# MohammadJohari/myslam

Hardware: AMD Instinct MI355X
Metric: ray.samples/s (render+bwd) (higher is better)
Workload: dtype f32; 1 GPU; BASELINE configs[1]: Replica room0 (synthetic), 4096 rays x 64 samples (56+8); mapping iteration: sample + render fwd + loss + bwd (planes+decoders), no optimiser; rays_of_the_job=4096, rays_this_rank=4096, samples_per_ray=64, plane_bytes=27147008, planes_layout=channels_last, parallelism=single GPU, launch=hipGraph replay of the captured iteration

## Files before the change

### include/eslam_hip.h

```cpp
#ifndef ESLAM_HIP_H
#define ESLAM_HIP_H

#include <stdint.h>

#ifdef __cplusplus
extern "C" {
#endif

#define ESLAM_ABI_VERSION 5
#define ESLAM_C_DIM 32
#define ESLAM_HIDDEN 16
#define ESLAM_FEAT (2 * ESLAM_C_DIM)
#define ESLAM_N_PLANES 12
#define ESLAM_MAX_SAMPLES 256
#define ESLAM_RAY_ORDERS 3
#define ESLAM_RAY_ORDER_WORDS(R) (ESLAM_RAY_ORDERS * (int64_t)(R) + 4)
#define ESLAM_N_DEC_PARAMS (2 * (16 * 64 + 16 + 16 * 16 + 16) + (1 * 16 + 1) + (3 * 16 + 3))

typedef void* eslam_stream_t;

typedef struct {
    const float* data;
    float* grad;
    int32_t h, w;
// ... 48 lines not shown
                           const uint32_t* rng_state, int64_t ray_offset, float* z_vals, eslam_stream_t stream);

int eslam_render_fwd(const eslam_plane_t* planes, const eslam_decoders_t* dec, const float* bound6_host,
                     const float* rays_o, const float* rays_d, const float* z_vals, int R, int S, float* depth,
                     float* rgb, float* sdf, float* raw_rgb, float* feat, const int32_t* ray_order,
                     uint32_t* rng_bump, eslam_stream_t stream);

int eslam_render_fwd_loss(const eslam_plane_t* planes, const eslam_decoders_t* dec, const float* bound6_host,
                          const float* rays_o, const float* rays_d, const float* z_vals, int R, int S, float* depth,
                          float* rgb, float* sdf, float* raw_rgb, float* feat, const int32_t* ray_order,
                          const float* gt_depth, const float* gt_color, double truncation, const float* weights5_host,
                          const uint8_t* ray_mask, float* scratch, float* acc, float* loss, uint32_t* rng_bump,
                          eslam_stream_t stream);

int eslam_planes_to_half(const eslam_plane_t* planes, eslam_stream_t stream);

int eslam_planes_relayout(const eslam_plane_t* src, const eslam_plane_t* dst, int field, eslam_stream_t stream);

int eslam_render_fwd_lowp(const eslam_plane_t* planes_f16, const eslam_decoders_t* dec, const float* bound6_host,
                          const float* rays_o, const float* rays_d, const float* z_vals, int R, int S, float* depth,
                          float* rgb, float* sdf, eslam_stream_t stream);

int eslam_ray_order(const float* rays_o, const float* rays_d, int R, int32_t* perm, eslam_stream_t stream);

int64_t eslam_bwd_workspace_bytes(int64_t n_points);

int eslam_render_bwd(const eslam_plane_t* planes, const eslam_decoders_t* dec, const float* bound6_host,
                     const float* rays_o, const float* rays_d, const float* z_vals, int R, int S,
                     const float* sdf, const float* raw_rgb, const float* feat, const float* g_depth,
                     const float* g_rgb, const float* g_sdf, float* g_dec, float* g_beta, float* g_rays_o,
                     float* g_rays_d, const int32_t* ray_order, void* workspace, eslam_stream_t stream);

int eslam_render_bwd_loss(const eslam_plane_t* planes, const eslam_decoders_t* dec, const float* bound6_host,
                          const float* rays_o, const float* rays_d, const float* z_vals, int R, int S,
                          const float* sdf, const float* raw_rgb, const float* feat, const float* depth,
                          const float* rgb, const float* gt_depth, const float* gt_color, double truncation,
                          const float* weights5_host, const uint8_t* ray_mask, const float* acc,
                          const float* upstream, float* loss_out, const float* g_depth, const float* g_rgb,
                          const float* g_sdf, float* g_dec, float* g_beta, float* g_rays_o, float* g_rays_d,
                          const int32_t* ray_order, void* workspace, eslam_stream_t stream);

int64_t eslam_saved_hidden_floats(int64_t R, int S);
int eslam_render_fwd_h(const eslam_plane_t* planes, const eslam_decoders_t* dec, const float* bound6_host,
                       const float* rays_o, const float* rays_d, const float* z_vals, int R, int S, float* depth,
                       float* rgb, float* sdf, float* raw_rgb, float* feat, const int32_t* ray_order,
                       uint32_t* rng_bump, float* hidden, eslam_stream_t stream);
// ... 224 lines not shown
```

### myslam_amd/_hip.py

```python
import ctypes
import os
import threading

import torch

_HERE = os.path.dirname(os.path.abspath(__file__))
LIB_PATH = os.environ.get("ESLAM_HIP_LIB") or os.path.join(_HERE, "lib", "libeslam_hip.so")

ABI_VERSION = 5
RAY_ORDERS = 3


def ray_order_words(R):
    return RAY_ORDERS * int(R) + 4
N_DEC_PARAMS = 2692
N_PLANES = 12


class PlaneDesc(ctypes.Structure):
    _fields_ = [("data", ctypes.c_void_p), ("grad", ctypes.c_void_p), ("h", ctypes.c_int32), ("w", ctypes.c_int32),
                ("stride_c", ctypes.c_int64), ("stride_y", ctypes.c_int64), ("stride_x", ctypes.c_int64),
                ("data_f16", ctypes.c_void_p)]


# ... 38 lines not shown
    "eslam_aabb_exit": (_i, [_vp, _vp, _i, _BP, _vp, _vp]),
    "eslam_sample_z": (_i, [_vp, _i, _i, _i, _d, _vp, _vp, _vp, _vp, _vp]),
    "eslam_importance_z": (_i, [_PP, _DP, _BP, _vp, _vp, _vp, _i, _i, _i, _vp, _vp, _vp, _vp, _vp]),
    "eslam_sample_z_all": (_i, [_PP, _DP, _BP, _vp, _vp, _vp, _i, _i, _i, _d, _vp, _vp, _vp, _vp, _vp, _vp, _vp]),
    "eslam_sample_z_all_rng": (_i, [_PP, _DP, _BP, _vp, _vp, _vp, _i, _i, _i, _d, _vp, _vp, _i, ctypes.c_uint64, _vp, _i64, _vp, _vp]),
    "eslam_loss_set_sizes": (_i, [_vp, _vp, _i, _i, _i, _d, _vp, _vp, _vp, _i, ctypes.c_uint64, _vp, _vp, _vp, _vp]),
    "eslam_mark_rays": (_i, [_PP, _BP, _vp, _vp, _vp, _i, _d, _vp, _i64, _vp, _vp]),
    "eslam_blocks_compact_scratch_words": (_i64, [_i64]),
    "eslam_blocks_compact": (_i, [_vp, _i64, _vp, _vp, _vp, _vp, _i, _vp]),
    "eslam_host_meta_alloc": (_i, [ctypes.POINTER(ctypes.c_void_p), ctypes.POINTER(ctypes.c_void_p)]),
    "eslam_host_meta_free": (_i, [_vp]),
    "eslam_shard_prologue": (_i, [_vp, _vp, _vp, _i64, _vp, _i64, _vp, _vp, _vp, _vp, _i, _i, _i, _d, _vp, _vp, _i, ctypes.c_uint64,
                                  _vp, _vp, _vp, _PP, _BP, _vp, _i64, _vp, _vp]),
    "eslam_blocks_pack_dev": (_i, [_vp, _vp, _vp, _i64, _vp, _i64, _i64, _vp, _vp, _vp]),
    "eslam_blocks_unpack_dev": (_i, [_vp, _vp, _vp, _i64, _vp, _i64, _i64, _vp, _vp]),
    "eslam_blocks_zero_dev": (_i, [_vp, _vp, _vp, _i64, _vp, _i64, _vp]),
    "eslam_render_fwd": (_i, [_PP, _DP, _BP, _vp, _vp, _vp, _i, _i, _vp, _vp, _vp, _vp, _vp, _vp, _vp, _vp]),
    "eslam_render_fwd_loss": (_i, [_PP, _DP, _BP, _vp, _vp, _vp, _i, _i, _vp, _vp, _vp, _vp, _vp, _vp, _vp, _vp, _d, _BP, _vp,
                                   _vp, _vp, _vp, _vp, _vp]),
    "eslam_planes_to_half": (_i, [_PP, _vp]),
    "eslam_planes_relayout": (_i, [_PP, _PP, _i, _vp]),
    "eslam_render_fwd_lowp": (_i, [_PP, _DP, _BP, _vp, _vp, _vp, _i, _i, _vp, _vp, _vp, _vp]),
    "eslam_ray_order": (_i, [_vp, _vp, _i, _vp, _vp]),
    "eslam_stream_wait": (_i, [_vp, _vp]),
    "eslam_zero_async": (_i, [_vp, _i64, _vp]),
    "eslam_bwd_workspace_bytes": (_i64, [_i64]),
    "eslam_render_bwd": (_i, [_PP, _DP, _BP, _vp, _vp, _vp, _i, _i, _vp, _vp, _vp, _vp, _vp, _vp, _vp, _vp, _vp, _vp,
                              _vp, _vp, _vp]),
    "eslam_render_bwd_loss": (_i, [_PP, _DP, _BP, _vp, _vp, _vp, _i, _i, _vp, _vp, _vp, _vp, _vp, _vp, _vp, _d, _BP, _vp, _vp,
                                   _vp, _vp, _vp, _vp, _vp, _vp, _vp, _vp, _vp, _vp, _vp, _vp]),
    "eslam_saved_hidden_floats": (_i64, [_i64, _i]),
    "eslam_render_fwd_h": (_i, [_PP, _DP, _BP, _vp, _vp, _vp, _i, _i, _vp, _vp, _vp, _vp, _vp, _vp, _vp, _vp, _vp]),
    "eslam_render_fwd_loss_h": (_i, [_PP, _DP, _BP, _vp, _vp, _vp, _i, _i, _vp, _vp, _vp, _vp, _vp, _vp, _vp, _vp, _d, _BP, _vp,
                                     _vp, _vp, _vp, _vp, _vp, _vp]),
    "eslam_render_bwd_h": (_i, [_PP, _DP, _BP, _vp, _vp, _vp, _i, _i, _vp, _vp, _vp, _vp, _vp, _vp, _vp, _vp, _vp, _vp,
                                _vp, _vp, _vp, _vp]),
    "eslam_render_bwd_loss_h": (_i, [_PP, _DP, _BP, _vp, _vp, _vp, _i, _i, _vp, _vp, _vp, _vp, _vp, _vp, _vp, _d, _BP, _vp, _vp,
                                     _vp, _vp, _vp, _vp, _vp, _vp, _vp, _vp, _vp, _vp, _vp, _vp, _vp]),
    "eslam_decode_fwd": (_i, [_PP, _DP, _BP, _vp, _i64, _i, _vp, _vp, _vp]),
    "eslam_sdf_grid": (_i, [_PP, _DP, _BP, _vp, _vp, _vp, _i64, _i64, _i64, _vp, _i, _i, _vp, _vp]),
    "eslam_mc_workspace_bytes": (_i64, [_i64, _i64, _i64]),
    "eslam_mc_count": (_i, [_vp, _i64, _i64, _i64, _f, _vp, _vp, _vp]),
    "eslam_mc_emit": (_i, [_vp, _i64, _i64, _i64, _f, ctypes.POINTER(_d), ctypes.POINTER(_d), _vp, _i64, _i64, _vp, _vp, _vp]),
    "eslam_mc_count_masked": (_i, [_vp, _vp, _i64, _i64, _i64, _f, _vp, _vp, _vp]),
    "eslam_tsdf_integrate": (_i, [_vp, _vp, _vp, _i64, _i64, _i64, ctypes.POINTER(_f), _f, _f, _vp, _vp, _vp, _vp, _i, _i, _i,
                                  _f, _f, _f, _f, _vp]),
# ... 254 lines not shown
```

### myslam_amd/csrc/eslam_sample.hip

```cpp
#include "eslam_decode_tile.h"

#pragma clang fp contract(off)

__device__ __forceinline__ void pixel_dir(float u, float v, float fx, float fy, float cx, float cy, float d[3]) {
    d[0] = __fdiv_rn(__fsub_rn(u, cx), fx);
    d[1] = -__fdiv_rn(__fsub_rn(v, cy), fy);
    d[2] = -1.0f;
}

__device__ __forceinline__ void rotate_dir(const float* __restrict__ c2w, const float d[3], float out[3]) {
#pragma unroll
    for (int j = 0; j < 3; ++j)
        out[j] = __fadd_rn(__fadd_rn(__fmul_rn(d[0], c2w[4 * j + 0]), __fmul_rn(d[1], c2w[4 * j + 1])),
                           __fmul_rn(d[2], c2w[4 * j + 2]));
}

__global__ void sample_rays_kernel(const int64_t* __restrict__ indices, int b, int n, int H0, int H1, int W0, int W1,
                                   int H, int W, float fx, float fy, float cx, float cy,
                                   const float* __restrict__ c2ws, const float* __restrict__ depths,
                                   const float* __restrict__ colors, float* __restrict__ rays_o,
                                   float* __restrict__ rays_d, float* __restrict__ depth, float* __restrict__ color) {
    const int i = blockIdx.x * blockDim.x + threadIdx.x;
    if (i >= b * n) return;
    const int img = i / n;
// ... 202 lines not shown
        zs[pos] = val;
    }
    WAVE_SYNC();
    for (int i = lane; i < S; i += WAVE)
        out[i] = t_rand ? jitter_one(zs, i, S, t_rand[(int64_t)ray * S + i])
                        : (rng.on && rng.perturb) ? jitter_one(zs, i, S, rng_uniform(rng, 0u, (rng.ray_offset + (uint32_t)ray) * (uint32_t)S + (uint32_t)i)) : zs[i];
}

__global__ __launch_bounds__(256) void sample_z_kernel(const float* __restrict__ gt_depth, int R, int n_strat,
                                                       int n_imp, float c15, float c3,
                                                       const float* __restrict__ t_free,
                                                       const float* __restrict__ t_surf,
                                                       const float* __restrict__ t_rand, float* __restrict__ z_vals) {
    __shared__ float zs_all[4][ESLAM_MAX_SAMPLES];
    const int lane = threadIdx.x & 63, wave = threadIdx.x >> 6;
    const int ray = blockIdx.x * 4 + wave;
    if (ray >= R) return;
    const float d = gt_depth[ray];
    if (!(d > 0.0f)) return;
    depth_guided_row(d, ray, n_strat, n_imp, c15, c3, t_free, t_surf, t_rand, z_vals + (int64_t)ray * (n_strat + n_imp), zs_all[wave], lane,
                     Rng{0u, 0u, false, false, 0u});
}

template <bool CL, bool WITH_DEPTH>
__global__ __launch_bounds__(256, 2) void importance_z_kernel(const PlaneSet planes, const eslam_decoders_t dec,
                                                           const Bound bnd, const float* __restrict__ rays_o,
                                                           const float* __restrict__ rays_d,
                                                           const float* __restrict__ gt_depth, int R, int n_strat,
                                                           int n_imp, const float* __restrict__ t_free,
                                                           const float* __restrict__ t_rand_uni,
                                                           const float* __restrict__ u_rand,
                                                           float* __restrict__ z_vals, float c15, float c3,
                                                           const float* __restrict__ t_surf,
                                                           const float* __restrict__ t_rand, const RngArg rng_arg) {
    const Rng rng = make_rng(rng_arg);
    __shared__ __attribute__((aligned(16))) float wlds[DEC_LDS];
    __shared__ float zu[ESLAM_MAX_SAMPLES];
    __shared__ float wt[ESLAM_MAX_SAMPLES];
    __shared__ float zn[ESLAM_MAX_SAMPLES];
    __shared__ float al[ESLAM_MAX_SAMPLES];
    const int lane = threadIdx.x & 63, wave = threadIdx.x >> 6;
    const int ray = blockIdx.x;
    const float d0 = gt_depth[ray];
    if (d0 > 0.0f) {
        if (WITH_DEPTH && wave == 0)
            depth_guided_row(d0, ray, n_strat, n_imp, c15, c3, t_free, t_surf, t_rand, z_vals + (int64_t)ray * (n_strat + n_imp), zu, lane, rng);
        return;
    }
    stage_decoder_weights_one(wlds, dec, 0, threadIdx.x, blockDim.x);
    const int r = lane & 15, q = lane >> 4;
    const int gp = gather_point<CL>(lane), gq = gather_piece<CL>(lane);
    const float beta = dec.beta[0];
    const int S = n_strat + n_imp;
    const float o[3] = {rays_o[3 * ray], rays_o[3 * ray + 1], rays_o[3 * ray + 2]};
    const float d[3] = {rays_d[3 * ray], rays_d[3 * ray + 1], rays_d[3 * ray + 2]};
    const float far = __fadd_rn(aabb_exit_dev(o, d, bnd), 0.01f);

    for (int i = threadIdx.x; i < n_strat; i += 256) {
        const float t = t_free[i];
        wt[i] = __fadd_rn(__fmul_rn(0.0f, __fsub_rn(1.0f, t)), __fmul_rn(far, t));
    }
    __syncthreads();
    for (int i = threadIdx.x; i < n_strat; i += 256)
        zu[i] = t_rand_uni ? jitter_one(wt, i, n_strat, t_rand_uni[(int64_t)ray * n_strat + i])
                           : (rng.on && rng.perturb) ? jitter_one(wt, i, n_strat, rng_uniform(rng, 1u, (rng.ray_offset + (uint32_t)ray) * (uint32_t)n_strat + (uint32_t)i)) : wt[i];
    __syncthreads();

    const int nblk = (n_strat + 15) >> 4;
#pragma unroll 1
    for (int b = wave; b < nblk; b += 4) {
        const int oz0 = opaque_zero(b);
        const float z = zu[min(16 * b + gp, n_strat - 1)];
// ... 60 lines not shown
    float* out_row = z_vals + (int64_t)ray * S;
    bool inversion = false;
    for (int i = lane; i + 1 < n_strat; i += WAVE) inversion |= !(zu[i] <= zu[i + 1]);
    const bool zu_sorted = __ballot(inversion) == 0ull;
    for (int i = lane; i < S; i += WAVE) {
        const float v = (i < n_strat) ? zu[i] : zn[i - n_strat];
        int pos = 0;
        if (zu_sorted) {
            if (i < n_strat) {
                pos = i;
                for (int j = 0; j < n_imp; ++j) pos += (zn[j] < v) ? 1 : 0;
            } else {
                const int j0 = i - n_strat;
                pos = count_le_sorted(zu, n_strat, v);
                for (int j = 0; j < n_imp; ++j) pos += (zn[j] < v || (zn[j] == v && j < j0)) ? 1 : 0;
            }
        } else {
            for (int k = 0; k < S; ++k) {
                const float o2 = (k < n_strat) ? zu[k] : zn[k - n_strat];
                pos += (o2 < v || (!(v < o2) && k < i)) ? 1 : 0;
            }
        }
        out_row[pos] = v;
    }
}


#include "eslam_loss_final.h"
#include "eslam_shard_dev.h"
struct SetSizesArgs {
    const float* gt_depth;
    const uint8_t* ray_mask;
    int R, n_strat, n_imp;
    float c15, c3;
    const float* t_free;
    const float* t_surf;
    const float* t_rand;
    RngArg rng;
    Trunc tr;
    unsigned* scratch;
    float* acc_out;
};
__device__ __forceinline__ void set_sizes_block(const SetSizesArgs& a, const int bid, const int nblocks) {
    const Rng rng = make_rng(a.rng);
    __shared__ float zs_all[4][ESLAM_MAX_SAMPLES];
    __shared__ float zo_all[4][ESLAM_MAX_SAMPLES];
// ... 163 lines not shown

extern "C" int eslam_importance_z(const eslam_plane_t* planes, const eslam_decoders_t* dec, const float* bound6_host,
                                  const float* rays_o, const float* rays_d, const float* gt_depth, int R, int n_strat,
                                  int n_imp, const float* t_free, const float* t_rand_uni, const float* u,
                                  float* z_vals, eslam_stream_t stream) {
    if (R <= 0) return 0;
    if (n_strat < 3 || n_imp < 0 || n_strat + n_imp > ESLAM_MAX_SAMPLES) {
        eslam_set_error("eslam_importance_z: n_strat=%d n_imp=%d unsupported", n_strat, n_imp);
        return 1;
    }
    if (!planes || !dec || !bound6_host || !rays_o || !rays_d || !gt_depth || !t_free || (n_imp > 0 && !u) || !z_vals) {
        eslam_set_error("eslam_importance_z: null argument");
        return 1;
    }
    if (eslam_validate_planes(planes, 0, 6)) return 1;
    PlaneSet ps;
    for (int i = 0; i < NPL; ++i) ps.p[i] = planes[i < 6 ? i : i - 6];
    const Bound bnd = make_bound(bound6_host);
    dim3 grid(R), block(256);
    eslam_prof_begin(PROF_IMPORTANCE_Z, (hipStream_t)stream);
    if (eslam_planes_channels_last(planes, 0, 6))
        hipLaunchKernelGGL((importance_z_kernel<true, false>), grid, block, 0, (hipStream_t)stream, ps, *dec, bnd, rays_o,
                           rays_d, gt_depth, R, n_strat, n_imp, t_free, t_rand_uni, u, z_vals, 0.0f, 0.0f,
                           (const float*)nullptr, (const float*)nullptr, RngArg{});
    else
        hipLaunchKernelGGL((importance_z_kernel<false, false>), grid, block, 0, (hipStream_t)stream, ps, *dec, bnd, rays_o,
                           rays_d, gt_depth, R, n_strat, n_imp, t_free, t_rand_uni, u, z_vals, 0.0f, 0.0f,
                           (const float*)nullptr, (const float*)nullptr, RngArg{});
    eslam_prof_end(PROF_IMPORTANCE_Z, (hipStream_t)stream);
    return eslam_check_launch("importance_z_kernel");
}

static int sample_z_all_impl(const char* who, const eslam_plane_t* planes, const eslam_decoders_t* dec,
                             const float* bound6_host, const float* rays_o, const float* rays_d, const float* gt_depth,
                             int R, int n_strat, int n_imp, double truncation, const float* t_free, const float* t_surf,
                             const float* t_rand, const float* t_rand_uni, const float* u, const RngArg rng,
                             float* z_vals, eslam_stream_t stream) {
    if (R <= 0) return 0;
    if (n_strat < 3 || n_imp < 0 || n_strat + n_imp > ESLAM_MAX_SAMPLES) {
        eslam_set_error("%s: n_strat=%d n_imp=%d unsupported", who, n_strat, n_imp);
        return 1;
    }
    if (!planes || !dec || !bound6_host || !rays_o || !rays_d || !gt_depth || !t_free ||
        (n_imp > 0 && ((!u && !rng.on) || !t_surf)) || !z_vals) {
        eslam_set_error("%s: null argument", who);
        return 1;
    }
    if ((int64_t)R * (n_strat + n_imp) >= ((int64_t)1 << 32)) {
        eslam_set_error("%s: batch too large", who);
        return 1;
    }
    if (eslam_validate_planes(planes, 0, 6)) return 1;
    PlaneSet ps;
    for (int i = 0; i < NPL; ++i) ps.p[i] = planes[i < 6 ? i : i - 6];
    const Bound bnd = make_bound(bound6_host);
    const float c15 = (float)(1.5 * truncation);
    const float c3 = (float)(3.0 * truncation);
    dim3 grid(R), block(256);
    eslam_prof_begin(PROF_SAMPLE_Z, (hipStream_t)stream);
    if (eslam_planes_channels_last(planes, 0, 6))
        hipLaunchKernelGGL((importance_z_kernel<true, true>), grid, block, 0, (hipStream_t)stream, ps, *dec, bnd, rays_o,
                           rays_d, gt_depth, R, n_strat, n_imp, t_free, t_rand_uni, u, z_vals, c15, c3, t_surf, t_rand, rng);
    else
        hipLaunchKernelGGL((importance_z_kernel<false, true>), grid, block, 0, (hipStream_t)stream, ps, *dec, bnd, rays_o,
                           rays_d, gt_depth, R, n_strat, n_imp, t_free, t_rand_uni, u, z_vals, c15, c3, t_surf, t_rand, rng);
    eslam_prof_end(PROF_SAMPLE_Z, (hipStream_t)stream);
    return eslam_check_launch("importance_z_kernel<with depth>");
}

extern "C" int eslam_sample_z_all(const eslam_plane_t* planes, const eslam_decoders_t* dec, const float* bound6_host,
                                  const float* rays_o, const float* rays_d, const float* gt_depth, int R, int n_strat,
                                  int n_imp, double truncation, const float* t_free, const float* t_surf,
                                  const float* t_rand, const float* t_rand_uni, const float* u, float* z_vals,
                                  eslam_stream_t stream) {
    return sample_z_all_impl("eslam_sample_z_all", planes, dec, bound6_host, rays_o, rays_d, gt_depth, R, n_strat, n_imp,
                             truncation, t_free, t_surf, t_rand, t_rand_uni, u, RngArg{}, z_vals, stream);
}

extern "C" int eslam_sample_z_all_rng(const eslam_plane_t* planes, const eslam_decoders_t* dec, const float* bound6_host,
                                      const float* rays_o, const float* rays_d, const float* gt_depth, int R, int n_strat,
                                      int n_imp, double truncation, const float* t_free, const float* t_surf, int perturb,
                                      uint64_t seed, const uint32_t* rng_state, int64_t ray_offset, float* z_vals,
                                      eslam_stream_t stream) {
    if (ray_offset < 0 || (ray_offset + (int64_t)(R > 0 ? R : 0)) * (n_strat + n_imp) >= ((int64_t)1 << 32)) {
        eslam_set_error("eslam_sample_z_all_rng: ray_offset %lld out of range", (long long)ray_offset);
        return 1;
    }
    RngArg rng;
// ... 88 lines not shown
```

### myslam_amd/csrc/eslam_scatter.hip

```cpp
#include <mutex>
#include <type_traits>
#include "eslam_decode_tile.h"
#include "eslam_dec_reduce.h"

#define SORT_MAX 8192
typedef float float2_t __attribute__((ext_vector_type(2)));

__device__ __forceinline__ unsigned spread3(unsigned v) {
    v &= 0x3FFu;
    v = (v | (v << 16)) & 0x030000FFu;
    v = (v | (v << 8)) & 0x0300F00Fu;
    v = (v | (v << 4)) & 0x030C30C3u;
    v = (v | (v << 2)) & 0x09249249u;
    return v;
}

#define ORD_BITS 5
#define ORD_CELLS (1 << (3 * ORD_BITS))
#define ORD_PER_THREAD (SORT_MAX / 1024)
__global__ __launch_bounds__(1024) void ray_order_kernel(const float* __restrict__ rays_o,
                                                         const float* __restrict__ rays_d, int R,
                                                         int* __restrict__ perm, int key_bits) {
    extern __shared__ __attribute__((aligned(16))) unsigned hist[];
    const int nwords = (1 << key_bits) >> 1;
    const int mbits = key_bits / 3;
    __shared__ float red[16][6];
    __shared__ float red2[16][11];
    __shared__ unsigned wsum[16];
    constexpr int NCAM_MAX = 32;
    __shared__ unsigned long long cam_bits[SORT_MAX / 64];
    __shared__ unsigned cam_before[SORT_MAX / 64 + 1];
    __shared__ float cam_dir[NCAM_MAX][3];
    __shared__ unsigned cam_ext[NCAM_MAX][2];
    const int tid = threadIdx.x, lane = tid & 63, wave = tid >> 6;
    if (tid < SORT_MAX / 64) cam_bits[tid] = 0ull;
    if (tid < NCAM_MAX) { cam_dir[tid][0] = cam_dir[tid][1] = cam_dir[tid][2] = 0.f; cam_ext[tid][0] = 0xFFFFFFFFu; cam_ext[tid][1] = 0u; }
    __syncthreads();
    const int base = blockIdx.x * SORT_MAX;
    const int n = min(SORT_MAX, R - base);
    const int orient = blockIdx.y;
    float* const fan = (float*)(perm + (size_t)ESLAM_RAY_ORDERS * R);
    perm += (size_t)orient * R;
    const int pa = orient == 2 ? 1 : 0, pb = orient == 0 ? 1 : 2;

    auto unit_dir = [&](int ray, float o[3], float d[3]) {
        const float dx = rays_d[3 * ray], dy = rays_d[3 * ray + 1], dz = rays_d[3 * ray + 2];
        const float inv = rsqrtf(fmaxf(dx * dx + dy * dy + dz * dz, 1e-20f));
        o[0] = rays_o[3 * ray]; o[1] = rays_o[3 * ray + 1]; o[2] = rays_o[3 * ray + 2];
        d[0] = dx * inv; d[1] = dy * inv; d[2] = dz * inv;
    };
    float lo[3] = {3.4e38f, 3.4e38f, 3.4e38f}, hi[3] = {-3.4e38f, -3.4e38f, -3.4e38f};
    float olo[3] = {3.4e38f, 3.4e38f, 3.4e38f}, ohi[3] = {-3.4e38f, -3.4e38f, -3.4e38f}, dsum[3] = {0.f, 0.f, 0.f};
    for (int i = tid; i < n; i += 1024) {
        float o[3], d[3];
        unit_dir(base + i, o, d);
#pragma unroll
        for (int a = 0; a < 3; ++a) {
            olo[a] = fminf(olo[a], o[a]); ohi[a] = fmaxf(ohi[a], o[a]);
            dsum[a] += d[a];
            const float p = o[a] + d[a];
            lo[a] = fminf(lo[a], p); hi[a] = fmaxf(hi[a], p);
        }
        bool first = i == 0;
        if (!first) {
            const float* po = rays_o + 3 * (size_t)(base + i - 1);
            first = po[0] != o[0] || po[1] != o[1] || po[2] != o[2];
        }
        const unsigned long long fb = __ballot(first);
        if (lane == 0) cam_bits[i >> 6] = fb;
    }
#pragma unroll
    for (int a = 0; a < 3; ++a) {
#pragma unroll
        for (int m = 32; m >= 1; m >>= 1) {
            lo[a] = fminf(lo[a], __shfl_xor(lo[a], m, WAVE));
            hi[a] = fmaxf(hi[a], __shfl_xor(hi[a], m, WAVE));
            olo[a] = fminf(olo[a], __shfl_xor(olo[a], m, WAVE));
            ohi[a] = fmaxf(ohi[a], __shfl_xor(ohi[a], m, WAVE));
            dsum[a] += __shfl_xor(dsum[a], m, WAVE);
        }
        if (lane == 0) {
            red[wave][a] = lo[a]; red[wave][3 + a] = hi[a];
            red2[wave][a] = olo[a]; red2[wave][3 + a] = ohi[a]; red2[wave][6 + a] = dsum[a];
        }
    }
    for (int i = tid; i < nwords; i += 1024) hist[i] = 0u;
    __syncthreads();
    if (wave == 0) {
        constexpr int NW = SORT_MAX / 64;
        const unsigned c0 = __popcll(cam_bits[2 * lane]), c1 = __popcll(cam_bits[2 * lane + 1]);
        const unsigned incl = wave_incl_sum_u(c0 + c1);
        cam_before[2 * lane] = incl - c0 - c1;
// ... 27 lines not shown
        for (int i = tid; i < n; i += 1024) {
            float o[3], d[3];
            unit_dir(base + i, o, d);
            const int c = camera_of(i);
            atomicAdd(&cam_dir[c][0], d[0]); atomicAdd(&cam_dir[c][1], d[1]); atomicAdd(&cam_dir[c][2], d[2]);
        }
        __syncthreads();
        auto angle = [&](int i, int& c) {
            float o[3], d[3];
            unit_dir(base + i, o, d);
            c = camera_of(i);
            const float ma = cam_dir[c][pa], mb = cam_dir[c][pb];
            return atan2f(ma * d[pb] - mb * d[pa], ma * d[pa] + mb * d[pb]);
        };
        for (int i = tid; i < n; i += 1024) {
            int c;
            const unsigned u = sortable(angle(i, c));
            atomicMin(&cam_ext[c][0], u);
            atomicMax(&cam_ext[c][1], u);
        }
        __syncthreads();
        const int cbits = 32 - __clz(ncam - 1);
        const int abits = key_bits - cbits;
        if (tid == 0 && blockIdx.x == 0) fan[orient] = 0.0f;
#pragma unroll
        for (int k = 0; k < ORD_PER_THREAD; ++k) {
            const int i = tid + k * 1024;
            if (i < n) {
                int c;
                const float ang = angle(i, c);
                const float l = unsortable(cam_ext[c][0]), h = unsortable(cam_ext[c][1]);
                const unsigned amax = (1u << abits) - 1u;
                const unsigned qa = min((unsigned)fmaxf((ang - l) * ((float)(1u << abits) / fmaxf(h - l, 1e-6f)), 0.f), amax);
                const unsigned kk = ((unsigned)c << abits) | qa;
                key[k] = kk;
                ticket[k] = (atomicAdd(&hist[kk >> 1], 1u << ((kk & 1u) * 16u)) >> ((kk & 1u) * 16u)) & 0xFFFFu;
            }
            __builtin_amdgcn_sched_barrier(0);
        }
    } else if (single) {
        const float mpa = mdir[pa] / mlen, mpb = mdir[pb] / mlen;
        auto azimuth = [&](int ray) {
            float o[3], d[3];
            unit_dir(ray, o, d);
            return atan2f(mpa * d[pb] - mpb * d[pa], mpa * d[pa] + mpb * d[pb]);
        };
        float blo = 3.4e38f, bhi = -3.4e38f;
        for (int i = tid; i < n; i += 1024) {
            const float u = azimuth(base + i);
            blo = fminf(blo, u); bhi = fmaxf(bhi, u);
        }
#pragma unroll
        for (int m = 32; m >= 1; m >>= 1) {
            blo = fminf(blo, __shfl_xor(blo, m, WAVE));
            bhi = fmaxf(bhi, __shfl_xor(bhi, m, WAVE));
        }
        if (lane == 0) { red2[wave][9] = blo; red2[wave][10] = bhi; }
        __syncthreads();
        float h = red2[0][10];
        blo = red2[0][9];
        for (int w = 1; w < 16; ++w) { blo = fminf(blo, red2[w][9]); h = fmaxf(h, red2[w][10]); }
        const float sc = (float)(1 << key_bits) / fmaxf(h - blo, 1e-6f);
        if (tid == 0 && blockIdx.x == 0) fan[orient] = h - blo;
#pragma unroll
        for (int k = 0; k < ORD_PER_THREAD; ++k) {
            const int i = tid + k * 1024;
            if (i < n) {
                const unsigned kk = min((unsigned)fmaxf((azimuth(base + i) - blo) * sc, 0.f), (1u << key_bits) - 1u);
                key[k] = kk;
                ticket[k] = (atomicAdd(&hist[kk >> 1], 1u << ((kk & 1u) * 16u)) >> ((kk & 1u) * 16u)) & 0xFFFFu;
            }
            __builtin_amdgcn_sched_barrier(0);
        }
    } else {
        if (tid == 0 && blockIdx.x == 0) fan[orient] = 0.0f;
        float scale[3];
#pragma unroll
        for (int a = 0; a < 3; ++a) {
            float l = red[0][a], h = red[0][3 + a];
            for (int w = 1; w < 16; ++w) { l = fminf(l, red[w][a]); h = fmaxf(h, red[w][3 + a]); }
            lo[a] = l;
            scale[a] = (float)(1 << mbits) / fmaxf(h - l, 1e-6f);
        }
#pragma unroll
        for (int k = 0; k < ORD_PER_THREAD; ++k) {
            const int i = tid + k * 1024;
            if (i < n) {
                float o[3], d[3];
                unit_dir(base + i, o, d);
                const unsigned qmax = (1u << mbits) - 1;
                const unsigned qx = min((unsigned)fmaxf((o[0] + d[0] - lo[0]) * scale[0], 0.f), qmax);
                const unsigned qy = min((unsigned)fmaxf((o[1] + d[1] - lo[1]) * scale[1], 0.f), qmax);
                const unsigned qz = min((unsigned)fmaxf((o[2] + d[2] - lo[2]) * scale[2], 0.f), qmax);
                const unsigned kk = spread3(qx) | (spread3(qy) << 1) | (spread3(qz) << 2);
                key[k] = kk;
                ticket[k] = (atomicAdd(&hist[kk >> 1], 1u << ((kk & 1u) * 16u)) >> ((kk & 1u) * 16u)) & 0xFFFFu;
            }
        }
// ... 436 lines not shown
            }
            WALK_HALF(gb, rec, g2 + 1, ebase)
        }
        rec = nxt;
    }
#undef LOAD_HALF
#undef WALK_HALF
    flush(false);
}

__global__ __launch_bounds__(256) void scatter_fixed_to_float_kernel(float* __restrict__ grad, long long* __restrict__ shadow,
                                                                     int64_t n) {
    for (int64_t i = (int64_t)blockIdx.x * 256 + threadIdx.x; i < n; i += (int64_t)gridDim.x * 256) {
        const long long v = shadow[i];
        if (v != 0) {
            grad[i] += (float)((double)v * (1.0 / 17592186044416.0));
            shadow[i] = 0;
        }
    }
}

int eslam_scatter_v2_init();

extern "C" int eslam_ray_order(const float* rays_o, const float* rays_d, int R, int32_t* perm, eslam_stream_t stream) {
    if (R <= 0) return 0;
    if (!rays_o || !rays_d || !perm) {
        eslam_set_error("eslam_ray_order: null argument");
        return 1;
    }
    hipStream_t st = (hipStream_t)stream;
    if (int rc = eslam_scatter_v2_init()) return rc;
    const int chunks = (R + SORT_MAX - 1) / SORT_MAX;
    const int n = R < SORT_MAX ? R : SORT_MAX;
    const int key_bits = n <= 1024 ? 12 : 14;
    hipLaunchKernelGGL(ray_order_kernel, dim3(chunks, ESLAM_RAY_ORDERS), dim3(1024), ((size_t)1 << key_bits) / 2 * sizeof(unsigned), st,
                       rays_o, rays_d, R, perm, key_bits);
    return eslam_check_launch("ray_order_kernel");
}

#define SC_SMALL_WGS 192
static int scatter_bundle_size(int per, int nunits, int* bm_out) {
    int bm = 2048;
    if (!eslam_deterministic()) {
        const int big = 2048 / per;
        const int nb = big > 0 ? (nunits + big - 1) / big : nunits;
        bm = (nb * NPL <= SC_SMALL_WGS && 1024 / per >= 1) ? 1024 : 2048;
    }
    *bm_out = bm;
    return bm / per;
}

extern "C" int eslam_scatter_bundle_samples(int64_t n, int S, int render) {
    if (n <= 0 || (render && (S <= 0 || S > 256))) return 0;
    int bm = 0;
    (void)scatter_bundle_size(render ? S : 64, render ? (int)n : (int)((n + 63) / 64), &bm);
    return bm;
}

bool eslam_scatter_can_reduce(bool render) {
    return render && !eslam_deterministic();
// ... 146 lines not shown
```

### myslam_amd/csrc/eslam_torch_ext.cpp

```cpp
#include <torch/extension.h>
#include <c10/hip/HIPGuard.h>
#include <c10/hip/HIPStream.h>
#include <hip/hip_runtime_api.h>

#include <cstdio>
#include <cstdlib>
#include <mutex>
#include <vector>

#include "../../include/eslam_hip.h"

namespace {

using torch::Tensor;
using torch::autograd::AutogradContext;
using torch::autograd::variable_list;

void check(int rc, const char* what) {
    TORCH_CHECK(rc == 0, what, " failed (rc=", rc, "): ", eslam_last_error());
}

struct Config {
    int64_t n_strat = 0, n_imp = 0;
    bool perturb = true;
// ... 126 lines not shown
            feat = at::empty({R * S, 128}, opt);
            if (io.saved_hidden && R > 0) hid = at::empty({eslam_saved_hidden_floats(R, (int)S)}, opt);
            perm = at::empty({planes_grad ? ESLAM_RAY_ORDER_WORDS(R) : 0}, opt.dtype(at::kInt));
        }
        if (io.relayout && R > 0) {
            auto cl = alloc_plane_grads(planes, Layout::channels_last);
            relayout(planes, cl.second, 0, st);
            planes = std::move(cl.second);
        }
        eslam_plane_t pd[ESLAM_N_PLANES];
        fill_planes(planes, nullptr, pd);
        eslam_decoders_t dd;
        fill_decoders(params, beta, &dd);

        std::vector<Tensor> grad_views;
        Tensor grad_flat;
        hipStream_t side = nullptr;
        if (planes_grad && R > 0) {
            side = side_stream(dev);
            auto gv = alloc_plane_grads(planes);
            grad_flat = gv.first;
            grad_views = std::move(gv.second);
            check(eslam_stream_wait(side, st), "eslam_stream_wait");
            check(eslam_zero_async(grad_flat.data_ptr<float>(), grad_flat.numel() * 4, side), "eslam_zero_async");
            check(eslam_ray_order(rays_o.data_ptr<float>(), rays_d.data_ptr<float>(), (int)R, perm.data_ptr<int32_t>(), side), "eslam_ray_order");
        }
        if (R > 0) {
            check(eslam_sample_z_all_rng(pd, &dd, io.cfg.bound_sample.data(), rays_o.data_ptr<float>(), rays_d.data_ptr<float>(),
                                         gd.data_ptr<float>(), (int)R, (int)io.cfg.n_strat, (int)io.cfg.n_imp, io.cfg.truncation,
                                         io.t_free.data_ptr<float>(), io.t_surf.data_ptr<float>(), io.cfg.perturb ? 1 : 0, io.seed,
                                         (const uint32_t*)io.rng_state.data_ptr<int32_t>(), io.ray_offset, z.data_ptr<float>(), st),
                  "eslam_sample_z_all_rng");
        }
        uint32_t* bump = (uint32_t*)io.rng_state.data_ptr<int32_t>();
        if (with_loss) {
            TORCH_CHECK(R > 0, "eslam_render_fwd_loss: empty batch");
            TORCH_CHECK(io.loss.gt_color.is_cuda() && io.loss.gt_color.scalar_type() == at::kFloat, "gt_color: expected a float32 tensor on the GPU");
            acc = io.loss.acc_out.defined() ? io.loss.acc_out : at::empty({16}, opt);
            value = at::empty({}, opt);
            const Tensor gc = io.loss.gt_color.contiguous();
            const uint8_t* mask = io.loss.ray_mask.defined() ? (const uint8_t*)io.loss.ray_mask.data_ptr() : nullptr;
            check(eslam_render_fwd_loss_h(pd, &dd, io.cfg.bound_decode.data(), rays_o.data_ptr<float>(), rays_d.data_ptr<float>(),
                                        z.data_ptr<float>(), (int)R, (int)S, depth.data_ptr<float>(), rgb.data_ptr<float>(),
                                        sdf.data_ptr<float>(), needs ? raw_rgb.data_ptr<float>() : nullptr,
                                        needs ? feat.data_ptr<float>() : nullptr, nullptr, gd.data_ptr<float>(), gc.data_ptr<float>(),
                                        io.cfg.truncation, io.loss.weights5.data(), mask, io.loss.scratch.data_ptr<float>(),
                                        acc.data_ptr<float>(), value.data_ptr<float>(), bump, hid.defined() ? hid.data_ptr<float>() : nullptr, st),
                  "eslam_render_fwd_loss");
// ... 250 lines not shown
```

### myslam_amd/ops.py

```python
import ctypes
import math
import os
import sys

import torch

from . import _hip

_const_cache = {}


def _cached(key, make):
    t = _const_cache.get(key)
    if t is None:
        t = make()
        _const_cache[key] = t
    return t


def beta_tensor(beta, device):
    if torch.is_tensor(beta):
        return beta
    dev = torch.device(device)
    return _cached(("beta", float(beta), dev.index), lambda: torch.full((1,), float(beta), device=dev))
# ... 184 lines not shown


_dec_param_cache = {}


_side_streams = {}


def ray_order_async(rays_o, rays_d, grad_planes=None):
    _hip.require_gpu_f32("rays_o", rays_o)
    _hip.require_gpu_f32("rays_d", rays_d)
    dev = rays_o.device
    ro, rd = _c(rays_o.detach()), _c(rays_d.detach())
    R = ro.shape[0]
    side = _side_streams.get(dev.index)
    if side is None:
        side = _side_streams[dev.index] = torch.cuda.Stream(device=dev)
    perm = torch.empty(_hip.ray_order_words(R), dtype=torch.int32, device=dev)
    pre = None
    if grad_planes is not None and _grad_sink is None and not _keep_layout:
        pre = _alloc_plane_grads(grad_planes, zero=False)
    _hip.stream_wait(dev, side, None)
    with _hip.on_device(dev):
        if pre is not None:
            _hip.check(_hip.lib().eslam_zero_async(_hip.ptr(pre[0]), pre[0].numel() * 4, ctypes.c_void_p(side.cuda_stream)),
                       "eslam_zero_async")
        _hip.check(_hip.lib().eslam_ray_order(_hip.ptr(ro), _hip.ptr(rd), R, _hip.ptr(perm),
                                              ctypes.c_void_p(side.cuda_stream)), "eslam_ray_order")
    perm.record_stream(side)
    for t, src in ((ro, rays_o), (rd, rays_d)):
        if t.data_ptr() != src.data_ptr():
            t.record_stream(side)
    return (perm, side) if pre is None else (perm, side, pre[1])


_fused_loss = None

SAVED_HIDDEN_DEFAULT = True
_saved_hidden = None


class saved_hidden:

    def __init__(self, on):
        self.on = None if on is None else bool(on)

    def __enter__(self):
        global _saved_hidden
        self.prev, _saved_hidden = _saved_hidden, self.on
        return self

# ... 1464 lines not shown
```

Baseline: 1.071 billion ray.samples/s.

## Fuse grad zeroing into ray-order kernel and compact importance sampling rays

The plane-gradient zeroing is folded into the ray-order launch as extra workgroups, so the separate memset launch on the side stream goes away. The ray-order kernel now loads rays in registers once, four at a time, and reuses the normalised directions for the azimuth pass instead of re-reading global memory. The depth-guided importance kernel is restructured. Rays with depth are handled four per workgroup, one per wave. Rays without depth are compacted per 1024-ray segment with ballots and a prefix sum, then spread over persistent workgroups, which avoids launching one 256-thread block per ray that mostly exits early. In exchange the importance kernel gains more indexing logic and a grid sized from the CU count.

```diff
diff --git a/include/eslam_hip.h b/include/eslam_hip.h
--- a/include/eslam_hip.h
+++ b/include/eslam_hip.h
@@ -94,6 +94,9 @@
                           float* rgb, float* sdf, eslam_stream_t stream);
 
 int eslam_ray_order(const float* rays_o, const float* rays_d, int R, int32_t* perm, eslam_stream_t stream);
+
+int eslam_ray_order_clear(const float* rays_o, const float* rays_d, int R, int32_t* perm, void* clear_ptr,
+                          int64_t clear_bytes, eslam_stream_t stream);
 
 int64_t eslam_bwd_workspace_bytes(int64_t n_points);
 
diff --git a/myslam_amd/_hip.py b/myslam_amd/_hip.py
--- a/myslam_amd/_hip.py
+++ b/myslam_amd/_hip.py
@@ -84,6 +84,7 @@
     "eslam_planes_relayout": (_i, [_PP, _PP, _i, _vp]),
     "eslam_render_fwd_lowp": (_i, [_PP, _DP, _BP, _vp, _vp, _vp, _i, _i, _vp, _vp, _vp, _vp]),
     "eslam_ray_order": (_i, [_vp, _vp, _i, _vp, _vp]),
+    "eslam_ray_order_clear": (_i, [_vp, _vp, _i, _vp, _vp, _i64, _vp]),
     "eslam_stream_wait": (_i, [_vp, _vp]),
     "eslam_zero_async": (_i, [_vp, _i64, _vp]),
     "eslam_bwd_workspace_bytes": (_i64, [_i64]),
diff --git a/myslam_amd/csrc/eslam_sample.hip b/myslam_amd/csrc/eslam_sample.hip
--- a/myslam_amd/csrc/eslam_sample.hip
+++ b/myslam_amd/csrc/eslam_sample.hip
@@ -248,32 +248,26 @@
                      Rng{0u, 0u, false, false, 0u});
 }
 
-template <bool CL, bool WITH_DEPTH>
-__global__ __launch_bounds__(256, 2) void importance_z_kernel(const PlaneSet planes, const eslam_decoders_t dec,
-                                                           const Bound bnd, const float* __restrict__ rays_o,
-                                                           const float* __restrict__ rays_d,
-                                                           const float* __restrict__ gt_depth, int R, int n_strat,
-                                                           int n_imp, const float* __restrict__ t_free,
-                                                           const float* __restrict__ t_rand_uni,
-                                                           const float* __restrict__ u_rand,
-                                                           float* __restrict__ z_vals, float c15, float c3,
-                                                           const float* __restrict__ t_surf,
-                                                           const float* __restrict__ t_rand, const RngArg rng_arg) {
-    const Rng rng = make_rng(rng_arg);
-    __shared__ __attribute__((aligned(16))) float wlds[DEC_LDS];
-    __shared__ float zu[ESLAM_MAX_SAMPLES];
-    __shared__ float wt[ESLAM_MAX_SAMPLES];
-    __shared__ float zn[ESLAM_MAX_SAMPLES];
-    __shared__ float al[ESLAM_MAX_SAMPLES];
+struct ImpLds {
+    float* wlds;
+    float* zu;
+    float* wt;
+    float* zn;
+    float* al;
+};
+template <bool CL>
+__device__ __forceinline__ void importance_row(const PlaneSet& planes, const eslam_decoders_t& dec, const Bound& bnd,
+                                               const float* __restrict__ rays_o, const float* __restrict__ rays_d,
+                                               const int ray, const int n_strat, const int n_imp,
+                                               const float* __restrict__ t_free, const float* __restrict__ t_rand_uni,
+                                               const float* __restrict__ u_rand, float* __restrict__ z_vals, const Rng& rng,
+                                               const ImpLds& L) {
+    float* const wlds = L.wlds;
+    float* const zu = L.zu;
+    float* const wt = L.wt;
+    float* const zn = L.zn;
+    float* const al = L.al;
     const int lane = threadIdx.x & 63, wave = threadIdx.x >> 6;
-    const int ray = blockIdx.x;
-    const float d0 = gt_depth[ray];
-    if (d0 > 0.0f) {
-        if (WITH_DEPTH && wave == 0)
-            depth_guided_row(d0, ray, n_strat, n_imp, c15, c3, t_free, t_surf, t_rand, z_vals + (int64_t)ray * (n_strat + n_imp), zu, lane, rng);
-        return;
-    }
-    stage_decoder_weights_one(wlds, dec, 0, threadIdx.x, blockDim.x);
     const int r = lane & 15, q = lane >> 4;
     const int gp = gather_point<CL>(lane), gq = gather_piece<CL>(lane);
     const float beta = dec.beta[0];
@@ -380,6 +374,90 @@
             }
         }
         out_row[pos] = v;
+    }
+}
+
+#define IMP_SEG 1024
+template <bool CL, bool WITH_DEPTH>
+__global__ __launch_bounds__(256, WITH_DEPTH ? 4 : 2) void importance_z_kernel(const PlaneSet planes, const eslam_decoders_t dec,
+                                                           const Bound bnd, const float* __restrict__ rays_o,
+                                                           const float* __restrict__ rays_d,
+                                                           const float* __restrict__ gt_depth, int R, int n_strat,
+                                                           int n_imp, const float* __restrict__ t_free,
+                                                           const float* __restrict__ t_rand_uni,
+                                                           const float* __restrict__ u_rand,
+                                                           float* __restrict__ z_vals, float c15, float c3,
+                                                           const float* __restrict__ t_surf,
+                                                           const float* __restrict__ t_rand, const RngArg rng_arg,
+                                                           const int row_wgs, const int seg_wgs) {
+    const Rng rng = make_rng(rng_arg);
+    __shared__ __attribute__((aligned(16))) float wlds[DEC_LDS];
+    __shared__ float zu[ESLAM_MAX_SAMPLES];
+    __shared__ float wt[ESLAM_MAX_SAMPLES];
+    __shared__ float zn[ESLAM_MAX_SAMPLES];
+    __shared__ float al[ESLAM_MAX_SAMPLES];
+    const ImpLds L = {wlds, zu, wt, zn, al};
+    const int lane = threadIdx.x & 63, wave = threadIdx.x >> 6;
+    if (!WITH_DEPTH) {
+        const int ray = blockIdx.x;
+        if (gt_depth[ray] > 0.0f) return;
+        stage_decoder_weights_one(wlds, dec, 0, threadIdx.x, blockDim.x);
+        importance_row<CL>(planes, dec, bnd, rays_o, rays_d, ray, n_strat, n_imp, t_free, t_rand_uni, u_rand, z_vals, rng, L);
+        return;
+    }
+    const int less_wgs = (int)gridDim.x - row_wgs;
+    if ((int)blockIdx.x >= less_wgs) {
+        const int ray = 4 * ((int)blockIdx.x - less_wgs) + wave;
+        if (ray >= R) return;
+        const float d0 = gt_depth[ray];
+        if (!(d0 > 0.0f)) return;
+        float* const zs = wave == 0 ? zu : wave == 1 ? wt : wave == 2 ? zn : al;
+        depth_guided_row(d0, ray, n_strat, n_imp, c15, c3, t_free, t_surf, t_rand, z_vals + (int64_t)ray * (n_strat + n_imp), zs, lane, rng);
+        return;
+    }
+    constexpr int NW = IMP_SEG / 64;
+    __shared__ unsigned long long less_bits[NW];
+    __shared__ unsigned less_before[NW + 1];
+    const int j = (int)blockIdx.x;
+    const int seg = j / seg_wgs, k = j - seg * seg_wgs;
+    const int seg_base = seg * IMP_SEG;
+    const int seg_n = min(IMP_SEG, R - seg_base);
+    if (seg_n <= 0 || k >= seg_n) return;
+    float dv[NW / 4];
+#pragma unroll
+    for (int m = 0; m < NW / 4; ++m) {
+        const int i = 64 * (wave + 4 * m) + lane;
+        dv[m] = i < seg_n ? gt_depth[seg_base + i] : 1.0f;
+    }
+#pragma unroll
+    for (int m = 0; m < NW / 4; ++m) {
+        const unsigned long long b = __ballot(!(dv[m] > 0.0f));
+        if (lane == 0) less_bits[wave + 4 * m] = b;
+    }
+    __syncthreads();
+    if (wave == 0) {
+        static_assert(NW <= 64 && NW % 4 == 0, "one ballot word per lane, the same number of words per wave");
+        const unsigned c = lane < NW ? (unsigned)__popcll(less_bits[lane]) : 0u;
+        const unsigned incl = wave_incl_sum_u(c);
+        if (lane < NW) less_before[lane] = incl - c;
+        if (lane == NW - 1) less_before[NW] = incl;
+    }
+    __syncthreads();
+    const int total = (int)less_before[NW];
+    if (k >= total) return;
+    stage_decoder_weights_one(wlds, dec, 0, threadIdx.x, blockDim.x);
+#pragma unroll 1
+    for (int idx = k; idx < total; idx += seg_wgs) {
+        int lo = 0, hi = NW - 1;
+        while (lo < hi) {
+            const int mid = (lo + hi + 1) >> 1;
+            if ((int)less_before[mid] <= idx) lo = mid; else hi = mid - 1;
+        }
+        unsigned long long bits = less_bits[lo];
+        for (int skip = idx - (int)less_before[lo]; skip > 0; --skip) bits &= bits - 1ull;
+        const int ray = seg_base + 64 * lo + (int)__builtin_ctzll(bits);
+        importance_row<CL>(planes, dec, bnd, rays_o, rays_d, ray, n_strat, n_imp, t_free, t_rand_uni, u_rand, z_vals, rng, L);
+        __syncthreads();
     }
 }
 
@@ -589,11 +667,11 @@
     if (eslam_planes_channels_last(planes, 0, 6))
         hipLaunchKernelGGL((importance_z_kernel<true, false>), grid, block, 0, (hipStream_t)stream, ps, *dec, bnd, rays_o,
                            rays_d, gt_depth, R, n_strat, n_imp, t_free, t_rand_uni, u, z_vals, 0.0f, 0.0f,
-                           (const float*)nullptr, (const float*)nullptr, RngArg{});
+                           (const float*)nullptr, (const float*)nullptr, RngArg{}, 0, 0);
     else
         hipLaunchKernelGGL((importance_z_kernel<false, false>), grid, block, 0, (hipStream_t)stream, ps, *dec, bnd, rays_o,
                            rays_d, gt_depth, R, n_strat, n_imp, t_free, t_rand_uni, u, z_vals, 0.0f, 0.0f,
-                           (const float*)nullptr, (const float*)nullptr, RngArg{});
+                           (const float*)nullptr, (const float*)nullptr, RngArg{}, 0, 0);
     eslam_prof_end(PROF_IMPORTANCE_Z, (hipStream_t)stream);
     return eslam_check_launch("importance_z_kernel");
 }
@@ -623,14 +701,30 @@
     const Bound bnd = make_bound(bound6_host);
     const float c15 = (float)(1.5 * truncation);
     const float c3 = (float)(3.0 * truncation);
-    dim3 grid(R), block(256);
+    static const int resident = [] {
+        int dev = 0, cus = 256;
+        if (hipGetDevice(&dev) == hipSuccess) (void)hipDeviceGetAttribute(&cus, hipDeviceAttributeMultiprocessorCount, dev);
+        return 4 * (cus > 0 ? cus : 256);
+    }();
+    const int row_wgs = (R + 3) / 4;
+    const int nseg = (R + IMP_SEG - 1) / IMP_SEG;
+    int seg_wgs = resident / nseg;
+    if (seg_wgs < 1) seg_wgs = 1;
+    if (seg_wgs > (R < IMP_SEG ? R : IMP_SEG)) seg_wgs = R < IMP_SEG ? R : IMP_SEG;
+    if ((int64_t)row_wgs + (int64_t)nseg * seg_wgs > 0x7FFFFFFF) {
+        eslam_set_error("%s: batch too large", who);
+        return 1;
+    }
+    dim3 grid(row_wgs + nseg * seg_wgs), block(256);
     eslam_prof_begin(PROF_SAMPLE_Z, (hipStream_t)stream);
     if (eslam_planes_channels_last(planes, 0, 6))
         hipLaunchKernelGGL((importance_z_kernel<true, true>), grid, block, 0, (hipStream_t)stream, ps, *dec, bnd, rays_o,
-                           rays_d, gt_depth, R, n_strat, n_imp, t_free, t_rand_uni, u, z_vals, c15, c3, t_surf, t_rand, rng);
+                           rays_d, gt_depth, R, n_strat, n_imp, t_free, t_rand_uni, u, z_vals, c15, c3, t_surf, t_rand, rng,
+                           row_wgs, seg_wgs);
     else
         hipLaunchKernelGGL((importance_z_kernel<false, true>), grid, block, 0, (hipStream_t)stream, ps, *dec, bnd, rays_o,
-                           rays_d, gt_depth, R, n_strat, n_imp, t_free, t_rand_uni, u, z_vals, c15, c3, t_surf, t_rand, rng);
+                           rays_d, gt_depth, R, n_strat, n_imp, t_free, t_rand_uni, u, z_vals, c15, c3, t_surf, t_rand, rng,
+                           row_wgs, seg_wgs);
     eslam_prof_end(PROF_SAMPLE_Z, (hipStream_t)stream);
     return eslam_check_launch("importance_z_kernel<with depth>");
 }
diff --git a/myslam_amd/csrc/eslam_scatter.hip b/myslam_amd/csrc/eslam_scatter.hip
--- a/myslam_amd/csrc/eslam_scatter.hip
+++ b/myslam_amd/csrc/eslam_scatter.hip
@@ -20,8 +20,19 @@
 #define ORD_PER_THREAD (SORT_MAX / 1024)
 __global__ __launch_bounds__(1024) void ray_order_kernel(const float* __restrict__ rays_o,
                                                          const float* __restrict__ rays_d, int R,
-                                                         int* __restrict__ perm, int key_bits) {
+                                                         int* __restrict__ perm, int key_bits, const int n_order,
+                                                         float* __restrict__ clear, const long long clear_words) {
     extern __shared__ __attribute__((aligned(16))) unsigned hist[];
+    if ((int)blockIdx.x >= n_order) {
+        const long long n16 = clear_words >> 2;
+        const long long stride = (long long)(gridDim.x - n_order) * 1024;
+        float4_t* const c4 = (float4_t*)clear;
+        const float4_t z4 = {0.f, 0.f, 0.f, 0.f};
+        for (long long i = (long long)((int)blockIdx.x - n_order) * 1024 + threadIdx.x; i < n16; i += stride) c4[i] = z4;
+        if ((int)blockIdx.x == n_order && (long long)threadIdx.x < (clear_words & 3)) clear[4 * n16 + threadIdx.x] = 0.f;
+        return;
+    }
+    const int chunk = (int)blockIdx.x / ESLAM_RAY_ORDERS;
     const int nwords = (1 << key_bits) >> 1;
     const int mbits = key_bits / 3;
     __shared__ float red[16][6];
@@ -36,38 +47,76 @@
     if (tid < SORT_MAX / 64) cam_bits[tid] = 0ull;
     if (tid < NCAM_MAX) { cam_dir[tid][0] = cam_dir[tid][1] = cam_dir[tid][2] = 0.f; cam_ext[tid][0] = 0xFFFFFFFFu; cam_ext[tid][1] = 0u; }
     __syncthreads();
-    const int base = blockIdx.x * SORT_MAX;
+    const int base = chunk * SORT_MAX;
     const int n = min(SORT_MAX, R - base);
-    const int orient = blockIdx.y;
+    const int orient = (int)blockIdx.x % ESLAM_RAY_ORDERS;
     float* const fan = (float*)(perm + (size_t)ESLAM_RAY_ORDERS * R);
     perm += (size_t)orient * R;
     const int pa = orient == 2 ? 1 : 0, pb = orient == 0 ? 1 : 2;
 
+    auto normalise = [](float dx, float dy, float dz, float d[3]) {
+        const float inv = rsqrtf(fmaxf(dx * dx + dy * dy + dz * dz, 1e-20f));
+        d[0] = dx * inv; d[1] = dy * inv; d[2] = dz * inv;
+    };
     auto unit_dir = [&](int ray, float o[3], float d[3]) {
-        const float dx = rays_d[3 * ray], dy = rays_d[3 * ray + 1], dz = rays_d[3 * ray + 2];
-        const float inv = rsqrtf(fmaxf(dx * dx + dy * dy + dz * dz, 1e-20f));
+        normalise(rays_d[3 * ray], rays_d[3 * ray + 1], rays_d[3 * ray + 2], d);
         o[0] = rays_o[3 * ray]; o[1] = rays_o[3 * ray + 1]; o[2] = rays_o[3 * ray + 2];
-        d[0] = dx * inv; d[1] = dy * inv; d[2] = dz * inv;
     };
     float lo[3] = {3.4e38f, 3.4e38f, 3.4e38f}, hi[3] = {-3.4e38f, -3.4e38f, -3.4e38f};
     float olo[3] = {3.4e38f, 3.4e38f, 3.4e38f}, ohi[3] = {-3.4e38f, -3.4e38f, -3.4e38f}, dsum[3] = {0.f, 0.f, 0.f};
-    for (int i = tid; i < n; i += 1024) {
-        float o[3], d[3];
-        unit_dir(base + i, o, d);
-#pragma unroll
-        for (int a = 0; a < 3; ++a) {
-            olo[a] = fminf(olo[a], o[a]); ohi[a] = fmaxf(ohi[a], o[a]);
-            dsum[a] += d[a];
-            const float p = o[a] + d[a];
-            lo[a] = fminf(lo[a], p); hi[a] = fmaxf(hi[a], p);
-        }
-        bool first = i == 0;
-        if (!first) {
-            const float* po = rays_o + 3 * (size_t)(base + i - 1);
-            first = po[0] != o[0] || po[1] != o[1] || po[2] != o[2];
-        }
-        const unsigned long long fb = __ballot(first);
-        if (lane == 0) cam_bits[i >> 6] = fb;
+    float ua[ORD_PER_THREAD], ub[ORD_PER_THREAD];
+    static_assert(ORD_PER_THREAD % 4 == 0, "rays are read four per thread at a time");
+#pragma unroll
+    for (int k0 = 0; k0 < ORD_PER_THREAD; k0 += 4) {
+        float ro[4][3], rd[4][3], rp[4][3];
+#pragma unroll
+        for (int k = 0; k < 4; ++k) {
+#pragma unroll
+            for (int a = 0; a < 3; ++a) ro[k][a] = rd[k][a] = rp[k][a] = 0.f;
+            ua[k0 + k] = ub[k0 + k] = 0.f;
+        }
+        if (k0 * 1024 >= n) continue;
+#pragma unroll
+        for (int k = 0; k < 4; ++k) {
+            const int i = tid + (k0 + k) * 1024;
+            if (i < n) {
+                const float* po = rays_o + 3 * (size_t)(base + i);
+                const float* pd = rays_d + 3 * (size_t)(base + i);
+#pragma unroll
+                for (int a = 0; a < 3; ++a) { ro[k][a] = po[a]; rd[k][a] = pd[a]; }
+                if (lane == 0 && i > 0) {
+#pragma unroll
+                    for (int a = 0; a < 3; ++a) rp[k][a] = po[a - 3];
+                }
+            }
+        }
+#pragma unroll
+        for (int k = 0; k < 4; ++k) {
+            const int i = tid + (k0 + k) * 1024;
+            float prev[3];
+#pragma unroll
+            for (int a = 0; a < 3; ++a) {
+                const float up = __shfl_up(ro[k][a], 1, WAVE);
+                prev[a] = lane == 0 ? rp[k][a] : up;
+            }
+            if (i < n) {
+                float d[3];
+                normalise(rd[k][0], rd[k][1], rd[k][2], d);
+                const float* o = ro[k];
+#pragma unroll
+                for (int a = 0; a < 3; ++a) {
+                    olo[a] = fminf(olo[a], o[a]); ohi[a] = fmaxf(ohi[a], o[a]);
+                    dsum[a] += d[a];
+                    const float p = o[a] + d[a];
+                    lo[a] = fminf(lo[a], p); hi[a] = fmaxf(hi[a], p);
+                }
+                ua[k0 + k] = orient == 2 ? d[1] : d[0];
+                ub[k0 + k] = orient == 0 ? d[1] : d[2];
+                const bool first = i == 0 || prev[0] != o[0] || prev[1] != o[1] || prev[2] != o[2];
+                const unsigned long long fb = __ballot(first);
+                if (lane == 0) cam_bits[i >> 6] = fb;
+            }
+        }
     }
 #pragma unroll
     for (int a = 0; a < 3; ++a) {
@@ -141,7 +190,7 @@
         __syncthreads();
         const int cbits = 32 - __clz(ncam - 1);
         const int abits = key_bits - cbits;
-        if (tid == 0 && blockIdx.x == 0) fan[orient] = 0.0f;
+        if (tid == 0 && chunk == 0) fan[orient] = 0.0f;
 #pragma unroll
         for (int k = 0; k < ORD_PER_THREAD; ++k) {
             const int i = tid + k * 1024;
@@ -159,15 +208,16 @@
         }
     } else if (single) {
         const float mpa = mdir[pa] / mlen, mpb = mdir[pb] / mlen;
-        auto azimuth = [&](int ray) {
-            float o[3], d[3];
-            unit_dir(ray, o, d);
-            return atan2f(mpa * d[pb] - mpb * d[pa], mpa * d[pa] + mpb * d[pb]);
-        };
+        float az[ORD_PER_THREAD];
         float blo = 3.4e38f, bhi = -3.4e38f;
-        for (int i = tid; i < n; i += 1024) {
-            const float u = azimuth(base + i);
-            blo = fminf(blo, u); bhi = fmaxf(bhi, u);
+#pragma unroll
+        for (int k = 0; k < ORD_PER_THREAD; ++k) {
+            az[k] = 0.f;
+            if (tid + k * 1024 < n) {
+                az[k] = atan2f(mpa * ub[k] - mpb * ua[k], mpa * ua[k] + mpb * ub[k]);
+                blo = fminf(blo, az[k]); bhi = fmaxf(bhi, az[k]);
+            }
+            __builtin_amdgcn_sched_barrier(0);
         }
 #pragma unroll
         for (int m = 32; m >= 1; m >>= 1) {
@@ -180,19 +230,18 @@
         blo = red2[0][9];
         for (int w = 1; w < 16; ++w) { blo = fminf(blo, red2[w][9]); h = fmaxf(h, red2[w][10]); }
         const float sc = (float)(1 << key_bits) / fmaxf(h - blo, 1e-6f);
-        if (tid == 0 && blockIdx.x == 0) fan[orient] = h - blo;
+        if (tid == 0 && chunk == 0) fan[orient] = h - blo;
 #pragma unroll
         for (int k = 0; k < ORD_PER_THREAD; ++k) {
             const int i = tid + k * 1024;
             if (i < n) {
-                const unsigned kk = min((unsigned)fmaxf((azimuth(base + i) - blo) * sc, 0.f), (1u << key_bits) - 1u);
+                const unsigned kk = min((unsigned)fmaxf((az[k] - blo) * sc, 0.f), (1u << key_bits) - 1u);
                 key[k] = kk;
                 ticket[k] = (atomicAdd(&hist[kk >> 1], 1u << ((kk & 1u) * 16u)) >> ((kk & 1u) * 16u)) & 0xFFFFu;
             }
-            __builtin_amdgcn_sched_barrier(0);
         }
     } else {
-        if (tid == 0 && blockIdx.x == 0) fan[orient] = 0.0f;
+        if (tid == 0 && chunk == 0) fan[orient] = 0.0f;
         float scale[3];
 #pragma unroll
         for (int a = 0; a < 3; ++a) {
@@ -675,20 +724,39 @@
 
 int eslam_scatter_v2_init();
 
+static int ray_order_launch(const char* who, const float* rays_o, const float* rays_d, int R, int32_t* perm, void* clear,
+                            int64_t clear_bytes, eslam_stream_t stream) {
+    if (clear_bytes < 0 || (clear_bytes > 0 && !clear) || ((uintptr_t)clear & 15) || (clear_bytes & 3)) {
+        eslam_set_error("%s: the buffer to clear must be 16-byte aligned and a multiple of 4 bytes long (%p, %lld bytes)", who, clear,
+                        (long long)clear_bytes);
+        return 1;
+    }
+    if (R <= 0 && clear_bytes == 0) return 0;
+    if (R > 0 && (!rays_o || !rays_d || !perm)) {
+        eslam_set_error("%s: null argument", who);
+        return 1;
+    }
+    hipStream_t st = (hipStream_t)stream;
+    if (int rc = eslam_scatter_v2_init()) return rc;
+    const int chunks = R > 0 ? (R + SORT_MAX - 1) / SORT_MAX : 0;
+    const int n = R < SORT_MAX ? R : SORT_MAX;
+    const int key_bits = n <= 1024 ? 12 : 14;
+    const int64_t want = (clear_bytes + 65535) / 65536;
+    const int n_clear = (int)(want < 256 ? want : 256);
+    const int n_order = chunks * ESLAM_RAY_ORDERS;
+    hipLaunchKernelGGL(ray_order_kernel, dim3(n_order + n_clear), dim3(1024), ((size_t)1 << key_bits) / 2 * sizeof(unsigned), st,
+                       rays_o, rays_d, R, perm, key_bits, n_order, (float*)clear, (long long)(clear_bytes >> 2));
+    return eslam_check_launch("ray_order_kernel");
+}
+
 extern "C" int eslam_ray_order(const float* rays_o, const float* rays_d, int R, int32_t* perm, eslam_stream_t stream) {
     if (R <= 0) return 0;
-    if (!rays_o || !rays_d || !perm) {
-        eslam_set_error("eslam_ray_order: null argument");
-        return 1;
-    }
-    hipStream_t st = (hipStream_t)stream;
-    if (int rc = eslam_scatter_v2_init()) return rc;
-    const int chunks = (R + SORT_MAX - 1) / SORT_MAX;
-    const int n = R < SORT_MAX ? R : SORT_MAX;
-    const int key_bits = n <= 1024 ? 12 : 14;
-    hipLaunchKernelGGL(ray_order_kernel, dim3(chunks, ESLAM_RAY_ORDERS), dim3(1024), ((size_t)1 << key_bits) / 2 * sizeof(unsigned), st,
-                       rays_o, rays_d, R, perm, key_bits);
-    return eslam_check_launch("ray_order_kernel");
+    return ray_order_launch("eslam_ray_order", rays_o, rays_d, R, perm, nullptr, 0, stream);
+}
+
+extern "C" int eslam_ray_order_clear(const float* rays_o, const float* rays_d, int R, int32_t* perm, void* clear_ptr,
+                                     int64_t clear_bytes, eslam_stream_t stream) {
+    return ray_order_launch("eslam_ray_order_clear", rays_o, rays_d, R, perm, clear_ptr, clear_bytes, stream);
 }
 
 #define SC_SMALL_WGS 192
diff --git a/myslam_amd/csrc/eslam_torch_ext.cpp b/myslam_amd/csrc/eslam_torch_ext.cpp
--- a/myslam_amd/csrc/eslam_torch_ext.cpp
+++ b/myslam_amd/csrc/eslam_torch_ext.cpp
@@ -172,8 +172,8 @@
             grad_flat = gv.first;
             grad_views = std::move(gv.second);
             check(eslam_stream_wait(side, st), "eslam_stream_wait");
-            check(eslam_zero_async(grad_flat.data_ptr<float>(), grad_flat.numel() * 4, side), "eslam_zero_async");
-            check(eslam_ray_order(rays_o.data_ptr<float>(), rays_d.data_ptr<float>(), (int)R, perm.data_ptr<int32_t>(), side), "eslam_ray_order");
+            check(eslam_ray_order_clear(rays_o.data_ptr<float>(), rays_d.data_ptr<float>(), (int)R, perm.data_ptr<int32_t>(),
+                                        grad_flat.data_ptr<float>(), grad_flat.numel() * 4, side), "eslam_ray_order_clear");
         }
         if (R > 0) {
             check(eslam_sample_z_all_rng(pd, &dd, io.cfg.bound_sample.data(), rays_o.data_ptr<float>(), rays_d.data_ptr<float>(),
diff --git a/myslam_amd/ops.py b/myslam_amd/ops.py
--- a/myslam_amd/ops.py
+++ b/myslam_amd/ops.py
@@ -230,11 +230,10 @@
         pre = _alloc_plane_grads(grad_planes, zero=False)
     _hip.stream_wait(dev, side, None)
     with _hip.on_device(dev):
-        if pre is not None:
-            _hip.check(_hip.lib().eslam_zero_async(_hip.ptr(pre[0]), pre[0].numel() * 4, ctypes.c_void_p(side.cuda_stream)),
-                       "eslam_zero_async")
-        _hip.check(_hip.lib().eslam_ray_order(_hip.ptr(ro), _hip.ptr(rd), R, _hip.ptr(perm),
-                                              ctypes.c_void_p(side.cuda_stream)), "eslam_ray_order")
+        _hip.check(_hip.lib().eslam_ray_order_clear(_hip.ptr(ro), _hip.ptr(rd), R, _hip.ptr(perm),
+                                                    None if pre is None else _hip.ptr(pre[0]),
+                                                    0 if pre is None else pre[0].numel() * 4,
+                                                    ctypes.c_void_p(side.cuda_stream)), "eslam_ray_order_clear")
     perm.record_stream(side)
     for t, src in ((ro, rays_o), (rd, rays_d)):
         if t.data_ptr() != src.data_ptr():
```

Result: faster. 1.101 billion ray.samples/s, median of 6 (+2.8%).
